# pliang279/factorized

Hardware: AMD Instinct MI355X
Metric: training samples/sec (MOSI-shape, T=20, 3 modalities) (higher is better)
Workload: dtype fp32; 1 GPU; MFM_KL_EF mosi canonical sizes, per-GPU B=32, T=20, D=325, train mode (fwd + joint loss + bwd + Adam), fp32 HIP; global_batch=32, seq_len=20, parallelism=dp1, params=477294, handover_failures=0, role_workgroups=True

## Files before the change

### factorized_amd/csrc/lstm_seq_small.hip

```cpp
#include "lstm_seq_small_dev.h"

namespace mfm {

#define MFM_SMALL_CASE(KK, BODY) case KK: BODY<KK, 4>(d, L.T, L.B, tile, lds); break;
#define MFM_SMALL_CASES(BODY) switch (d.hk4) { MFM_HK4_CASES(MFM_SMALL_CASE, BODY) default: break; }

template <bool BWD>
__global__ __launch_bounds__(1024) void lstm_seq_small_kernel(const SeqLaunch L) {
  extern __shared__ __attribute__((aligned(16))) float lds[];
  const int bid = blockIdx.x;
  MFM_SEQ_BLOCK_LSTM(L, bid, di)
  const SeqDev& d = L.d[di];
  const int tile = bid - d.block_begin;
  if (BWD) {
    MFM_SMALL_CASES(small_bwd_body)
  } else {
    MFM_SMALL_CASES(small_fwd_body)
  }
}

template <bool BWD, int R, int KS, int K0, int K1, int K2, int K3, int K4 = 0, int K5 = 0, bool BF = false>
__global__ __launch_bounds__(KS == 16 ? 1024 : 512) void lstm_seq_small_kernel4(const SeqLaunch L) {
  extern __shared__ __attribute__((aligned(16))) float lds[];
  const int bid = blockIdx.x;
// ... 73 lines not shown
template <bool BWD, int K0, int K1, int K2, int K3>
__global__ __launch_bounds__(1024) void lstm_seq_small_fold_kernel(const SeqLaunch L, const LatentDev LD, const float* __restrict__ params,
                                                                   float* __restrict__ grads) {
  extern __shared__ __attribute__((aligned(16))) float lds[];
  const int bid = blockIdx.x;
  if constexpr (!BWD) {
    if (L.n_img > 0 && bid >= L.img_begin) { wt_img_write(L.img, L.n_img, bid - L.img_begin, L.n_img_blocks); return; }
  }
  MFM_SEQ_BLOCK_LSTM(L, bid, di)
  const SeqDev& d = L.d[di];
  const int tile = bid - d.block_begin;
  if constexpr (BWD) {
    latent_bwd_row_body<false>(LD, params, grads, tile, di, lds);
    sync_stores();
  }
  MFM_TUPLE4(if (BWD) small_bwd_body<KQ, 1, 16>(d, L.T, L.B, tile, lds); else small_fwd_body<KQ, 1>(d, L.T, L.B, tile, lds))
  if constexpr (!BWD) {
    sync_stores();
    latent_fwd_row_body<false>(LD, params, tile, di, lds, true);
  }
}

template <int K0, int K1, int K2, int K3>
__global__ __launch_bounds__(1024) void lstm_seq_small_foldproj_kernel(const SeqLaunch L, const LatentDev LD, const ProjRole PR,
                                                                       const float* __restrict__ params) {
  extern __shared__ __attribute__((aligned(16))) float lds[];
  const int bid = blockIdx.x;
  const unsigned epoch = ho_epoch(PR.epoch, PR.tick);
  LSTAMP(0, 0);
  if (bid < PR.n_role) { proj_role_body(L, PR, epoch, lds); LSTAMP(0, 15); return; }
  MFM_SEQ_BLOCK_LSTM(L, bid, di)
  const SeqDev& d = L.d[di];
  const int tile = bid - d.block_begin;
  const unsigned* flg = PR.flags + (int64_t)di * L.T * PROJ_ROLE_FLAGS;
  const int ncb = PR.e[di].ncb;
  const bool pre = PR.lat_pre != 0;
  float* seq_lds = lds;
  if (pre) {
    latent_fwd_row_body<false>(LD, params, tile, di, lds, true, 1);
    seq_lds = lds + latent_fwd_lds_floats(LD.rec_size);
  }
  const float* h_lds = nullptr;
  MFM_TUPLE4(h_lds = small_fwd_body<KQ, 1, true>(d, L.T, L.B, tile, seq_lds, flg, epoch, ncb, PR.ctl))
  if (threadIdx.x < 64) {
    unsigned fv[4];
#pragma unroll
    for (int e = 0; e < 4; ++e) fv[e] = proj_flags_load(PR.flags + (int64_t)e * L.T * PROJ_ROLE_FLAGS, PR.e[e].ncb);
#pragma unroll
    for (int e = 0; e < 4; ++e) proj_flags_wait(PR.flags + (int64_t)e * L.T * PROJ_ROLE_FLAGS, fv[e], epoch, PR.e[e].ncb, PR.ctl);
  }
  LSTAMP(0, 9);
  if (pre) {
    LSTAMP(0, 8);
    latent_fwd_row_body<false>(LD, params, tile, di, lds, true, 2, h_lds, PR.lat_tail ? LD.tail_from : MFM_LAT_MAXSTAGES);
  } else {
    sync_stores();
    LSTAMP(0, 8);
    latent_fwd_row_body<false>(LD, params, tile, di, lds, true);
  }
  LSTAMP_W(0, 15);
}

template <int K0, int K1, int K2, int K3>
__global__ __launch_bounds__(1024) void lstm_seq_small_folddw_kernel(const SeqLaunch L, const LatentDev LD, const DwRole DR,
                                                                     const float* __restrict__ params, float* __restrict__ grads) {
  extern __shared__ __attribute__((aligned(16))) float lds[];
  const int bid = blockIdx.x;
  const unsigned epoch = ho_epoch(DR.epoch, DR.tick);
  LSTAMP(4, 0);
  if (bid >= 4 * L.B) {
    typedef __attribute__((address_space(4))) const char kchar;
    const char* kargs = (const char*)(kchar*)__builtin_amdgcn_kernarg_segment_ptr();
    dw_role_body(DR, epoch, lds, reinterpret_cast<const int*>(kargs + sizeof(SeqLaunch) + sizeof(LatentDev)));
    LSTAMP_W(4, 15);
    return;
  }
// ... 172 lines not shown
    if (!L.d[i].wt_img) return MFM_ERR_UNSUPPORTED;
  const int head_begin = lay_out_blocks(L, L.B), total = head_begin + 4 * L.B;
  const size_t lds_bytes = std::max(chain_lds_bytes(LD, true), small_lds_bytes(L, true, 1));
  if (lds_bytes > 160 * 1024) return MFM_ERR_UNSUPPORTED;
  return seq_launch_kernel(lstm_seq_small_decbwd_head_kernel<26, 6, 6>, "lstm_seq_small_decbwd_head_kernel", dim3(total), dim3(1024), lds_bytes, stream,
                           nullptr, L, LD, params, grads, head_begin);
}

bool seq_small_foldproj_supported(int T, int B, const int* h, const int* k, int n_enc) {
  if (opt_disabled("MFM_PROJ_FOLD") || !fold_enabled()) return false;
  if (n_enc != 4 || T < 1 || B < 1 || B > PROJ_ROLE_CB) return false;
  if (device_cus() - 4 * B < PROJ_ROLE_SLOTS) return false;
  int slots = 0, kmax = 0;
  for (int e = 0; e < 4; ++e) {
    if (k[e] < 1 || k[e] > 128 * PROJ_ROLE_MAXG) return false;
    slots += 4 * round_up(h[e], 16) / PROJ_ROLE_CB;
    if (4 * round_up(h[e], 16) / PROJ_ROLE_CB > PROJ_ROLE_FLAGS) return false;
    kmax = std::max(kmax, k[e]);
  }
  if (slots > PROJ_ROLE_SLOTS) return false;
  const int ks = proj_role_kstride(kmax);
  return ((size_t)2 * PROJ_ROLE_CB * ks + 16 * PROJ_ROLE_PW) * sizeof(float) <= 160 * 1024;
}

int seq_small_foldproj_launch(SeqLaunch& L, const LatentDev& LD, ProjRole& PR, const float* params, hipStream_t stream) {
  if (!seq_is_tuple(L, kEncHk4, 4, 0) || !chain_rows_match(LD, L.B)) return MFM_ERR_UNSUPPORTED;
  int hh[4], kk[4];
  for (int i = 0; i < 4; ++i) { hh[i] = L.d[i].h; kk[i] = PR.e[i].k; }
  if (!seq_small_foldproj_supported(L.T, L.B, hh, kk, 4)) return MFM_ERR_UNSUPPORTED;
  LSTAMP_BIND();
  int n_role = (device_cus() - 4 * L.B) / PROJ_ROLE_SLOTS * PROJ_ROLE_SLOTS;
  if (const char* e = opt_get("MFM_PROJ_FOLD_ROLES")) { const int v = atoi(e) / PROJ_ROLE_SLOTS * PROJ_ROLE_SLOTS; if (v >= PROJ_ROLE_SLOTS) n_role = v; }
  PR.n_role = n_role; PR.groups = n_role / PROJ_ROLE_SLOTS;
  int kmax = 0, cb = 0;
  for (int i = 0; i < 4; ++i) {
    kmax = std::max(kmax, PR.e[i].k);
    PR.e[i].cb_begin = cb; PR.e[i].ncb = 4 * L.d[i].Hp / PROJ_ROLE_CB;
    cb += PR.e[i].ncb;
  }
  PR.kstride = proj_role_kstride(kmax);
  const int total = lay_out_blocks(L, L.B, n_role);
  const size_t role = ((size_t)2 * PROJ_ROLE_CB * PR.kstride + 16 * PROJ_ROLE_PW) * sizeof(float);
  size_t lds_bytes = std::max(small_lds_bytes(L, false, 1), std::max(chain_lds_bytes(LD, false), role));
  PR.lat_pre = 0;
  if (!opt_disabled("MFM_LATENT_PRELOAD")) {
    bool direct = true;
    for (int i = 0; i < 4; ++i) direct = direct && (L.d[i].h & 3) == 0;
    const size_t side = chain_lds_bytes(LD, false) + small_lds_bytes(L, false, 1, true);
    if (direct && side <= 160 * 1024) { PR.lat_pre = 1; lds_bytes = std::max(side, role); }
  }
  if (!PR.lat_pre) PR.lat_tail = 0;
  if (lds_bytes > 160 * 1024) return MFM_ERR_UNSUPPORTED;
  return seq_launch_kernel(lstm_seq_small_foldproj_kernel<8, 2, 20, 30>, "lstm_seq_small_foldproj_kernel", dim3(total), dim3(1024), lds_bytes, stream, nullptr,
                           L, LD, PR, params);
}

int seq_small_fold_launch(SeqLaunch& L, bool bwd, const LatentDev& LD, const float* params, float* grads, hipStream_t stream) {
  if (!fold_enabled() || !seq_is_tuple(L, kEncHk4, 4, 0) || !chain_rows_match(LD, L.B)) return MFM_ERR_UNSUPPORTED;
  if (!((long)L.count * L.B < 6L * device_cus())) return MFM_ERR_UNSUPPORTED;
  int max_threads = 1024;
  for (int i = 0; i < 4; ++i)
    if (8 * L.d[i].Hp > max_threads) max_threads = 8 * L.d[i].Hp;
  int total = lay_out_blocks(L, L.B);
  L.n_img_blocks = 0;
  if (!bwd && L.n_img > 0) total = add_img_writers(L, total);
  const size_t lds_bytes = std::max(small_lds_bytes(L, bwd, 1), chain_lds_bytes(LD, bwd));
  if (lds_bytes > 160 * 1024) return MFM_ERR_UNSUPPORTED;
  return seq_launch_kernel(bwd ? lstm_seq_small_fold_kernel<true, 8, 2, 20, 30> : lstm_seq_small_fold_kernel<false, 8, 2, 20, 30>, "lstm_seq_small_fold_kernel",
                           dim3(total), dim3(max_threads), lds_bytes, stream, nullptr, L, LD, params, grads);
}

// ... 2 lines not shown
```

### factorized_amd/csrc/lstm_seq_small_dev.h

```cpp
#pragma once
#include <stdlib.h>

#include <algorithm>
#include <type_traits>

#include "internal.h"
#include "latent_row_dev.h"
#include "lstm_seq_dev.h"
#include "proj_role_dev.h"
#include "dw_role_dev.h"
#include "lstamp.h"

namespace mfm {

__device__ __forceinline__ void sync_stores() {
  asm volatile("s_waitcnt vmcnt(0)" ::: "memory");
  __syncthreads();
}

#ifndef MFM_SEQ_STAMP
#define MFM_SEQ_STAMP 0
#endif
#ifndef MFM_SEQ_LATE_WRITEOUT
#define MFM_SEQ_LATE_WRITEOUT 0
// ... 62 lines not shown
  } else {
    for (int i = tid; i < n; i += nt) panel[i] = (mode == 2) ? a[i] + b2[i] : a[i];
  }
}

__device__ __forceinline__ void stage_gates2(const SeqDev& d, int mode, int g, float* __restrict__ panel, int tid, int nt) {
  const int n = d.h * d.h;
  if ((n & 3) != 0) {
    stage_gate(d, mode, g, panel, tid, nt);
    stage_gate(d, mode, g + 1, panel + n, tid, nt);
    return;
  }
  const int n4 = n >> 2;
  const f32x4* a4 = reinterpret_cast<const f32x4*>((mode == 0 ? d.w_hh : d.w_ih) + (int64_t)g * n);
  const f32x4* b4 = reinterpret_cast<const f32x4*>(d.w_hh + (int64_t)g * n);
  f32x4* p4 = reinterpret_cast<f32x4*>(panel);
  for (int base = tid; base < 2 * n4; base += 8 * nt) {
    f32x4 v[8];
#pragma unroll
    for (int u = 0; u < 8; ++u) v[u] = a4[min(base + u * nt, 2 * n4 - 1)];
    if (mode == 2) {
#pragma unroll
      for (int u = 0; u < 8; ++u) v[u] += b4[min(base + u * nt, 2 * n4 - 1)];
    }
#pragma unroll
    for (int u = 0; u < 8; ++u)
      if (base + u * nt < 2 * n4) p4[base + u * nt] = v[u];
  }
}

typedef __bf16 bf16x2_t __attribute__((ext_vector_type(2)));
template <int KQ, int R, bool FLG = false, bool BF = false, bool REC = true, bool HS = false>
__device__ __forceinline__ const float* small_fwd_body(const SeqDev& d, const int T, const int B, const int tile, float* lds,
                                               const unsigned* flg = nullptr, const unsigned epoch = 0, const int ncb = 0,
                                               const HoCtl ctl = HoCtl{nullptr, nullptr, nullptr, 5000000ll, 1u},
                                               const int64_t hs_step = 0) {
  constexpr int HK = 4 * KQ;
  constexpr int HKB = (HK + 15) / 16 * 16;
  constexpr int NTH = 8 * HKB;
  constexpr int NXL = (4 * R + 7) / 8;
  constexpr int NOS = (6 * R + 7) / 8;
  const int tid = threadIdx.x, nt = blockDim.x;
  const int q = tid & 3, gp = (tid >> 2) & 1, u = tid >> 3;
  const int h = d.h, Hp = d.Hp;
  const bool dec = d.is_dec != 0;
  const bool uact = u < Hp;
  const int myrow = q & (R - 1);
  const bool rowner = q < R;
  const int b0 = tile * R;
  const int b = b0 + myrow;

  constexpr int NM = HKB / 16;
  constexpr int NWR = (R == 1) ? 4 * NM : KQ;
  constexpr int HX = (R == 1) ? HKB : HK;
  static_assert(!BF || R == 1, "bf16 dot products: one-row tiles only");
  static_assert(!HS || (!REC && !BF), "h-only record: fp32 inference bodies");
  float* hbuf = lds;
  __bf16* hb16 = reinterpret_cast<__bf16*>(lds);
  float* panel = lds + 2 * HKB * R;
  float* obuf = panel;
  float* xbuf = obuf + 2 * 6 * HKB * R;

  float w[2][NWR];
  bf16x2_t wp[2][BF ? NWR / 2 : 1];
  auto pack_w = [&]() {
    if constexpr (BF) {
#pragma unroll
      for (int gl = 0; gl < 2; ++gl)
#pragma unroll
        for (int j = 0; j < NWR / 2; ++j) wp[gl][j] = bf16x2_t{(__bf16)w[gl][2 * j], (__bf16)w[gl][2 * j + 1]};
    }
  };
  auto load_w = [&](int mode) {
    if constexpr (R == 1) {
      const float* fimg = mode == 2 ? d.wf_img : (mode == 1 ? d.wf1_img : nullptr);
      if (fimg) {
        const f32x4* img = reinterpret_cast<const f32x4*>(fimg) + (tid < NTH ? tid : 0);
#pragma unroll
        for (int gl = 0; gl < 2; ++gl)
#pragma unroll
          for (int m = 0; m < NM; ++m) {
            const f32x4 v = img[(gl * NM + m) * NTH];
#pragma unroll
            for (int i = 0; i < 4; ++i) w[gl][4 * m + i] = (tid < NTH) ? v[i] : 0.0f;
          }
        pack_w();
        return;
      }
      if ((h & 3) == 0) {
// ... 37 lines not shown
  load_w(dec ? 1 : 0);
  LSTAMP_W(dec ? 1 : 0, 1);

  float gxb[2] = {0.f, 0.f};
  if (dec && u < h) {
#pragma unroll
    for (int gl = 0; gl < 2; ++gl) gxb[gl] = d.b_ih[(2 * gp + gl) * h + u] + d.b_hh[(2 * gp + gl) * h + u];
  }
  if (dec) {
    for (int idx = tid; idx < HX * R; idx += nt) {
      const int k = idx / R, br = b0 + (idx % R);
      const float v = (k < h && br < B) ? d.h_init[(int64_t)br * d.ld_init + k] : 0.0f;
      if constexpr (BF) hb16[idx] = (__bf16)v; else hbuf[idx] = v;
    }
  }

  const int64_t row4 = 4 * (int64_t)Hp;
  const int64_t gstep = (int64_t)B * row4, sstep = (int64_t)B * Hp;
  const gfloat* xp[NXL];
  int xl[NXL];
  bool xok[NXL];
  float xpf[NXL];
#pragma unroll
  for (int i = 0; i < NXL; ++i) {
    const int e = tid + i * NTH;
    xok[i] = !dec && tid < NTH && e < 4 * HKB * R;
    const int ec = xok[i] ? e : 0;
    const int sr = ec / HKB, unit = ec % HKB, r = sr % R, g = sr / R;
    xp[i] = (const gfloat*)d.gates + ((int64_t)min(b0 + r, B - 1) * 4 + g) * Hp + unit;
    xl[i] = (g * HKB + unit) * R + r;
    xpf[i] = 0.0f;
  }
  const bool fetch_wave = FLG && !dec && (tid & ~63) < 4 * HKB * R && (tid & ~63) < NTH;
  unsigned fv = 0;
  if (!dec) {
    if constexpr (FLG) {
      if (fetch_wave) {
        const int t1 = (T > 1) ? 1 : 0;
        proj_flags_wait(flg, proj_flags_load(flg, ncb), epoch, ncb, ctl);
        proj_flags_wait(flg + t1 * PROJ_ROLE_FLAGS, proj_flags_load(flg + t1 * PROJ_ROLE_FLAGS, ncb), epoch, ncb, ctl);
        fv = proj_flags_load(flg + min(2, T - 1) * PROJ_ROLE_FLAGS, ncb);
      }
    }
#pragma unroll
    for (int i = 0; i < NXL; ++i) {
      float v0;
      if constexpr (FLG) { v0 = ld_agent((const float*)xp[i]); xpf[i] = ld_agent((const float*)xp[i] + ((T > 1) ? gstep : 0)); }
      else { v0 = xp[i][0]; xpf[i] = xp[i][(T > 1) ? gstep : 0]; }
      if (xok[i]) xbuf[xl[i]] = v0;
    }
  }
  gfloat* const p_gates = pin_s(d.gates);
  gfloat* const p_cs = pin_s(d.cs);
  gfloat* const p_hs = pin_s(d.hs);
  gfloat* op[NOS];
  int64_t ostr[NOS];
  int ol[NOS];
  bool ook[NOS];
#pragma unroll
  for (int i = 0; i < NOS; ++i) {
    const int e = tid + i * NTH;
    const bool in = tid < NTH && e < 6 * HKB * R;
    const int ec = in ? e : 0;
    const int sr = ec / HKB, unit = ec % HKB, r = sr % R, sl = sr / R;
    ook[i] = in && (b0 + r < B);
    const int br = min(b0 + r, B - 1);
    op[i] = sl < 4 ? p_gates + ((int64_t)br * 4 + sl) * Hp + unit : (sl == 4 ? p_cs : p_hs) + (int64_t)br * Hp + unit;
    ostr[i] = sl < 4 ? gstep : sstep;
    ol[i] = (sl * HKB + unit) * R + r;
  }
  gfloat* hs_p = p_hs;
  int hs_l = 0;
  bool hs_ok = false;
  if constexpr (HS) {
    const int r = tid / HKB, unit = tid - r * HKB;
    hs_ok = tid < HKB * R && b0 + r < B;
    hs_p = p_hs + (int64_t)min(b0 + r, B - 1) * Hp + (hs_ok ? unit : 0);
    hs_l = (hs_ok && unit < HX) ? unit * R + r : -1;
  }
  const int ucl = min(u, HKB - 1);
  const int my_o = (2 * gp * HKB + ucl) * R + myrow;
  const float sc0 = gp ? 2.0f : 1.0f;
// ... 67 lines not shown
            acc[1][0] = fmaf(w[1][4 * m + i], hv[m][i], acc[1][0]);
          }
#if MFM_SEQ_STAMP == 2
        asm volatile("s_memtime %0" : "=s"(st1), "+v"(acc[0][0]), "+v"(acc[1][0]) :: "memory");
#endif
      }
    } else if (dec || t > 0) {
      const float* hb = hbuf + cur * (HK * R) + q * R;
      constexpr int RING = (KQ < 4) ? KQ : 4;
      RowVec<R> ring[RING];
#pragma unroll
      for (int j = 0; j < RING; ++j) ring[j] = ld_rows<R>(hb + 4 * R * j);
#pragma unroll
      for (int j = 0; j < KQ; ++j) {
        const RowVec<R> hv = ring[j % RING];
        if (j + RING < KQ) ring[j % RING] = ld_rows<R>(hb + 4 * R * (j + RING));
#pragma unroll
        for (int gl = 0; gl < 2; ++gl)
#pragma unroll
          for (int r = 0; r < R; ++r) acc[gl][r] = fmaf(w[gl][j], hv.v[r], acc[gl][r]);
      }
    }
    if (REC && MFM_SEQ_LATE_WRITEOUT && pend) {
#pragma unroll
      for (int i = 0; i < NOS; ++i) {
        if (ook[i]) *op[i] = rprev[i];
        op[i] += ostr[i];
      }
    }
    pend = true;
    float xn[NXL];
#pragma unroll
    for (int i = 0; i < NXL; ++i) xn[i] = 0.0f;
    if (!dec) {
      const int64_t off = (int64_t)min(t + 2, T - 1) * gstep;
      if constexpr (FLG) {
        if (fetch_wave) {
          proj_flags_wait(flg + min(t + 2, T - 1) * PROJ_ROLE_FLAGS, fv, epoch, ncb, ctl);
#pragma unroll
          for (int i = 0; i < NXL; ++i) xn[i] = ld_agent((const float*)xp[i] + off);
          fv = proj_flags_load(flg + min(t + 3, T - 1) * PROJ_ROLE_FLAGS, ncb);
        }
      } else {
#pragma unroll
        for (int i = 0; i < NXL; ++i) xn[i] = xp[i][off];
      }
    }
    float mine[2];
#pragma unroll
    for (int gl = 0; gl < 2; ++gl) {
#pragma unroll
      for (int r = 0; r < R; ++r) {
        float v = acc[gl][r];
        v += dpp_f<DPP_QUAD_XOR1>(v);
        v += dpp_f<DPP_QUAD_XOR2>(v);
        acc[gl][r] = v;
      }
      mine[gl] = sel_row<R>(acc[gl], myrow) + (gl ? gx1 : gx0);
    }
    const float a0 = act_scaled(mine[0], sc0);
    const float a1 = act_sigmoid(mine[1]);
    const float p0 = dpp_xor4(a0), p1 = dpp_xor4(a1);
    const float gf = gp ? p1 : a1, go = gp ? a1 : p1;
    c = fmaf(gf, c, a0 * p0);
    float hv = go * act_tanh(c);
#if MFM_SEQ_STAMP == 3
    asm volatile("s_memtime %0" : "=s"(st1), "+v"(hv), "+v"(c) :: "memory");
#endif
    if (uact && rowner) {
      if constexpr (REC) {
        float* ob = obuf + par * (6 * HKB * R) + my_o;
        ob[0] = a0; ob[HKB * R] = a1;
        ob[(4 - gp) * HKB * R] = gp ? hv : c;
      }
      if (gp == 0 && u < HX) {
        const float hn = (b < B) ? hv : 0.0f;
        if constexpr (BF) hb16[(cur ^ 1) * HX + u] = (__bf16)hn; else hbuf[(cur ^ 1) * (HX * R) + u * R + myrow] = hn;
      }
    }
    if (!dec) {
#pragma unroll
      for (int i = 0; i < NXL; ++i)
        if (xok[i]) xbuf[(par ^ 1) * (4 * HKB * R) + xl[i]] = xpf[i];
    }
#if MFM_SEQ_STAMP == 4
    asm volatile("s_waitcnt lgkmcnt(0)" ::: "memory");
    st1 = seq_clock();
#endif
    lds_barrier();
#if MFM_SEQ_STAMP == 5
    st1 = seq_clock();
#endif
#if MFM_SEQ_STAMP
    if (MFM_SEQ_STAMP != 6 && t >= 1) { asm volatile("s_waitcnt lgkmcnt(0)" ::: "memory"); st_sum += st1 - st0; }
#endif
    if (REC && !MFM_SEQ_LATE_WRITEOUT) {
#pragma unroll
      for (int i = 0; i < NOS; ++i) {
        if (ook[i]) *op[i] = obuf[par * (6 * HKB * R) + ol[i]];
        op[i] += ostr[i];
      }
      pend = false;
    }
    if constexpr (HS) {
      if (hs_ok) *hs_p = hs_l >= 0 ? hbuf[(cur ^ 1) * (HX * R) + hs_l] : 0.0f;
      hs_p += hs_step;
    }
#pragma unroll
    for (int i = 0; i < NXL; ++i) xpf[i] = xn[i];
    cur ^= 1;
  };
  auto flush = [&](const int t_last) {
    if (!REC || !pend) return;
#pragma unroll
    for (int i = 0; i < NOS; ++i) {
      if (ook[i]) *op[i] = obuf[(t_last & 1) * (6 * HKB * R) + ol[i]];
      op[i] += ostr[i];
    }
    pend = false;
  };
  if (dec) {
    step(0);
    flush(0);
    LSTAMP(1, 3);
    if (T > 1) {
      __syncthreads();
      load_w(2);
      LSTAMP_W(1, 4);
      for (int t = 1; t < T; ++t) step(t);
      flush(T - 1);
    }
  } else {
    for (int t = 0; t < T; ++t) step(t);
    flush(T - 1);
  }
  LSTAMP(dec ? 1 : 0, 7);
#if MFM_SEQ_STAMP
  __syncthreads();
  if (blockIdx.x == 0 && (tid & 63) == 0 && T > 2) {
    const int nsteps = (MFM_SEQ_STAMP == 6) ? T - 2 : T - 1;
    p_cs[(int64_t)(T - 1) * sstep + (tid >> 6)] = (float)((double)st_sum / (double)nsteps);
  }
// ... 357 lines not shown
```

### factorized_amd/csrc/plan_build.hip

```cpp
#include "plan_internal.h"

namespace mfm {

PIdx pidx_for(int variant) {
  PIdx p;
  memset(&p, 0xff, sizeof(p));
  p.enc[0] = 0; p.enc[1] = 6; p.enc[2] = 12;
  p.dec[0] = 18; p.dec[1] = 24; p.dec[2] = 30;
  if (variant == 0) {
    p.enc[3] = 36;
    p.to_z[3] = 42; p.to_lv[3] = 44; p.to_z[0] = 46; p.to_z[1] = 48; p.to_z[2] = 50;
    p.to_lv[0] = 52; p.to_lv[1] = 54; p.to_lv[2] = 56;
    p.zf1[3] = 58; p.zf2[3] = 60; p.zf1[0] = 62; p.zf2[0] = 64; p.zf1[1] = 66; p.zf2[1] = 68; p.zf1[2] = 70; p.zf2[2] = 72;
    p.y_f1 = 74; p.y_f2 = 76; p.count = 78;
    return p;
  }
  p.mfl[0] = 36; p.mfl[1] = 40; p.mfl[2] = 44;
  p.att1_1 = 48; p.att1_2 = 50; p.att2_1 = 52; p.att2_2 = 54; p.g1_1 = 56; p.g1_2 = 58; p.g2_1 = 60; p.g2_2 = 62;
  p.to_z[3] = 68;
  int next = 70;
  if (variant == 1) {
    p.to_lv[3] = 70; p.to_z[0] = 72; p.to_z[1] = 74; p.to_z[2] = 76; p.to_lv[0] = 78; p.to_lv[1] = 80; p.to_lv[2] = 82;
    next = 84;
  }
// ... 344 lines not shown
      }
      L.bias_tab = fits ? 1 : 0;
    }
    L.bias_n = 0;
    for (int ch = 0; ch < L.nch && L.bias_tab; ++ch) {
      int cnt = 0;
      for (int i = 0; i < L.nops; ++i) if (L.nch == 1 || P->lat_ops[i].chain == ch) cnt += P->lat_ops[i].N;
      L.bias_n = std::max(L.bias_n, cnt);
    }
    L.pre = 0;
    if (const char* e = opt_get("MFM_LATENT_PRE")) L.pre = (atoi(e) != 0 && L.nch > 1 && L.nstages <= 6) ? 1 : 0;
    for (int ch = 0; ch < L.nch && L.pre; ++ch)
      for (int st = 0; st < L.nstages; ++st)
        if (L.nitems_fwd_c[ch][st] > 512 || L.nitems_bwd_c[ch][st] > 512) L.pre = 0;
    L.row_threads = MFM_LAT_ROW_THREADS;
    if (L.nch > 1) {
      int mx = 0;
      for (int ch = 0; ch < L.nch; ++ch)
        for (int st = 0; st < L.nstages; ++st) mx = std::max(mx, std::max(L.nitems_fwd_c[ch][st], L.nitems_bwd_c[ch][st]));
      int in_sum = 0;
      for (int e = 0; e < 4; ++e) in_sum += L.enc_n[e];
      if (mx <= 512 && in_sum <= 512) L.row_threads = 512;
    }
    if (L.nch > 1)
      for (int st = 0; st < L.nstages; ++st) {
        int sn = 0, sk = 0;
        for (int i = L.stage_begin[st]; i < L.stage_begin[st + 1]; ++i) { sn += P->lat_ops[i].N; sk += P->lat_ops[i].K; }
        L.nitems_fwd[st] = 4 * sn; L.nitems_bwd[st] = 4 * sk;
      }
  }

  P->lat_ops_off = carve(cur, (int64_t)(sizeof(P->lat_ops) / (sizeof(float))));
  P->pf_flags = (V == 0) ? carve(cur, (int64_t)4 * P->T * PROJ_ROLE_FLAGS) : -1;
  if ((long)(P->n_enc > 3 ? P->n_enc : 3) * c.B < 6L * device_cus() && !P->seq_bf16) {
    for (int i = 0; i < P->n_enc + 3; ++i) {
      const int hh = i < P->n_enc ? P->enc[i].h : P->dec[i - P->n_enc].h;
      if (hh > MFM_SEQ_MAX_RESIDENT_H) continue;
      const int64_t HKB = round_up(4 * round_up(cdiv(hh, 4), 2), 16);
      P->wt_img[i] = carve(cur, 4 * HKB * HKB);
      if (i >= P->n_enc && (hh & 3) == 0) { P->wf_img[i - P->n_enc] = carve(cur, 4 * HKB * HKB); P->wf_img[3 + i - P->n_enc] = carve(cur, 4 * HKB * HKB); }
    }
  }
  if (V == 0 && c.B <= DWR_ROWS) {
    P->dw_flags = carve(cur, (int64_t)4 * P->T * DWR_ROWS + 4 * DWR_ROWS);
    P->dw_table = carve(cur, (int64_t)DWR_TABLE_CAP * 4);
  }
  P->lat_items_off = carve(cur, (int64_t)P->lat_items.size());
  P->lat_grd = carve(cur, (int64_t)c.B * rs);
  P->lat_rec = carve(cur, (int64_t)c.B * rs);
  P->lat_seed = (V == 2) ? carve(cur, (int64_t)c.B * rs) : -1;
  {
    long minb = 48;
    if (const char* e = opt_get("MFM_MMD_GEMM_MINB")) minb = atol(e);
    P->mmd_scr = (V == 2 && minb > 0 && c.B >= minb && c.B <= 8192) ? carve(cur, mmd_scratch_floats(c.B, 4)) : -1;
  }
  if (V != 0) P->dh_last[3] = carve(cur, (int64_t)c.B * P->nzy);
  P->yhat = carve(cur, (int64_t)c.B * c.output_dim);
  P->ones = carve(cur, TB);
  P->losses = carve(cur, 64);
  P->ws_floats = cur;
  return MFM_OK;
}

}
```

### factorized_amd/csrc/plan_forward.hip

```cpp
#include "plan_internal.h"

namespace mfm {

__global__ void tick_kernel(unsigned long long* t64, unsigned* t32) {
  if (threadIdx.x == 0 && blockIdx.x == 0) {
    if (t64) *t64 += 1ull;
    if (t32) *t32 += 1u;
  }
}
__global__ void guard_propagate_kernel(const unsigned* status, float* guard) {
  if (threadIdx.x == 0 && blockIdx.x == 0 && *status != 0u) *guard = __builtin_nanf("");
}
bool stream_capturing(hipStream_t s) {
  hipStreamCaptureStatus st = hipStreamCaptureStatusNone;
  if (hipStreamIsCapturing(s, &st) != hipSuccess) { (void)hipGetLastError(); return false; }
  return st == hipStreamCaptureStatusActive;
}

MfmSeqDesc seq_desc(const MfmPlan* P, const SeqBuf& sb, int pbase, const float* params, float* W, bool dec) {
  MfmSeqDesc d;
  memset(&d, 0, sizeof(d));
  d.gates = W + sb.gates; d.hs = W + sb.hs; d.cs = W + sb.cs;
  d.w_ih = params + P->off[pbase + W_IH];
  d.w_hh = params + P->off[pbase + W_HH];
// ... 54 lines not shown
      PL.ngroups = P->n_enc;
      for (int e = 0; e < P->n_enc; ++e) {
        const SeqBuf& sb = P->enc[e];
        const int pb = P->enc_p[e];
        PanelGroup& G = PL.g[e];
        G.w = params + P->off[pb + W_IH]; G.ldw = P->enc_d[e];
        G.bias = params + P->off[pb + B_IH]; G.bias2 = params + P->off[pb + B_HH];
        G.n = 4 * sb.Hp; G.seg = sb.Hp; G.seg_valid = sb.h; G.k_off = P->enc_xoff[e]; G.k_len = P->enc_d[e];
      }
      const int rc0 = proj_pack_prepare(PL, P->pj, W + P->pj_wimg, W + P->pj_bimg, &PJD);
      if (rc0 != MFM_OK) return rc0;
      pjp = &PJD; P->pj_pack_call = P->calls;
    }
    if (st16 && train && !(xhat_out && (xhat_out[0] || xhat_out[1] || xhat_out[2]))) {
      DecFc1LargeLaunch FLp;
      memset(&FLp, 0, sizeof(FLp));
      FLp.n_items = 3; FLp.rows = (int)TB;
      for (int m = 0; m < 3; ++m) {
        DecFc1LargeItem& I = FLp.it[m];
        I.w = params + P->off[P->dec_p[m] + FC_W]; I.d = P->dec_d[m]; I.h = P->dec[m].h; I.Hp = P->dec[m].Hp;
        I.ld_dxhat = P->dxh_ld[m]; I.ldx = P->D; I.wimg = W + P->fc1_wimg[m];
      }
      if (dec_fc1_large_uses_wimg(FLp)) {
        const int rc0 = fc1_pack_prepare(FLp, &FCA);
        if (rc0 != MFM_OK) return rc0;
        fcp = &FCA; P->fc1_pack_call = P->calls;
      }
    }
    RUN(K_PACK, pack_all_launch(&PKL, pjp, fcp, s));
  }

  bool proj_in_fold = false;
  const bool capturing = stream_capturing(s);
  if (V == 0 && !seq_bf16 && !st16 && P->n_enc == 4 && P->fold_state >= 0 && P->projfold_state >= 0 && P->pf_flags >= 0 &&
      P->opt_handover && TB * P->D < ((int64_t)1 << 28)) {
    int hh[4], kk[4];
    for (int e = 0; e < 4; ++e) { hh[e] = P->enc[e].h; kk[e] = P->enc_d[e]; }
    proj_in_fold = seq_small_foldproj_supported(T, B, hh, kk, 4);
    if (!proj_in_fold) P->projfold_state = -1;
  }
  auto run_f0 = [&]() -> int {
    MfmGemmDesc g[6];
    memset(g, 0, sizeof(g));
    for (int e = 0; e < P->n_enc; ++e) {
      const SeqBuf& sb = P->enc[e];
      const int pb = P->enc_p[e];
      MfmGemmDesc& d = g[e];
      d.a = x + P->enc_xoff[e]; d.a_sm = P->D; d.a_sk = 1; d.a_sz = 0;
      d.b = params + P->off[pb + W_IH]; d.b_sz = (int64_t)sb.h * P->enc_d[e]; d.b_sn = P->enc_d[e]; d.b_sk = 1;
      d.c = W + sb.gates; d.c_sz = sb.Hp; d.ldc = 4 * (int64_t)sb.Hp;
      d.c_bf16 = st16 ? 1 : 0;
      d.bias = params + P->off[pb + B_IH]; d.bias2 = params + P->off[pb + B_HH]; d.bias_sz = sb.h;
      d.m = (int)TB; d.n = sb.Hp; d.n_valid = sb.h; d.k = P->enc_d[e]; d.batch = 4; d.split_k = 1;
      d.alpha = 1.0f;
    }
    const char* pe = opt_get("MFM_PANEL_MINROWS");
    const bool panel_forced = pe && TB >= atol(pe);
    const bool panel = (pe ? panel_forced : TB >= 16L * device_cus()) && P->n_enc <= MFM_PANEL_MAXG && (int64_t)TB * P->D < ((int64_t)1 << 29);
    if (panel || (st16 && P->proj16)) {
      PanelLaunch PL;
      memset(&PL, 0, sizeof(PL));
      PL.a = x; PL.lda = P->D; PL.M = (int)TB; PL.K = P->D;
      for (int e = 0; e < P->n_enc; ++e) {
        const SeqBuf& sb = P->enc[e];
        const int pb = P->enc_p[e];
        PanelGroup& G = PL.g[PL.ngroups++];
        G.w = params + P->off[pb + W_IH]; G.ldw = P->enc_d[e];
// ... 43 lines not shown
          I.w_hh = sum ? params + P->off[pb + W_HH] : nullptr; I.w_ih = params + P->off[pb + W_IH];
          I.img = W + P->wf_img[sum ? m : 3 + m]; I.h = P->dec[m].h;
          I.HKB = round_up(4 * round_up(cdiv(P->dec[m].h, 4), 2), 16);
          I.fwd = 1;
        }
      }
    }
  }
  LatentDev L = P->lat;
  {
    L.ops = reinterpret_cast<const LatOp*>(W + P->lat_ops_off);
    L.items_fwd = reinterpret_cast<const int*>(W + P->lat_items_off);
    L.items_bwd = L.items_fwd + (size_t)4 * MFM_LAT_MAXSTAGES * MFM_LAT_ROW_THREADS * 4;
    for (int e = 0; e < 4; ++e) {
      if (e == 3 && V != 0) { L.enc_h[e] = W + P->zyin; L.enc_ld[e] = P->nzy; continue; }
      L.enc_h[e] = st16 ? W + P->h_last[e] : W + P->enc[e].hs + (int64_t)(T - 1) * B * P->enc[e].Hp;
      L.enc_ld[e] = P->enc[e].Hp;
    }
    for (int m = 0; m < 3; ++m) { L.dec_init[m] = W + P->dec_init[m]; L.dec_ld[m] = P->dec_h[m]; }
    L.rec = W + P->lat_rec;
    L.yhat_out = yhat_out ? yhat_out : W + P->yhat;
    L.y = y; L.losses = losses; L.train = train;
    L.seed = seed * 0x9E3779B97F4A7C15ull + P->calls * 0xD1B54A32D192ED03ull;
    L.tick = reinterpret_cast<const unsigned long long*>(P->tick_ptr(W));
  }
  bool folded = false;
  if (proj_in_fold) {
    MfmSeqDesc q[4];
    for (int e = 0; e < 4; ++e) q[e] = seq_desc(P, P->enc[e], P->enc_p[e], params, W, false);
    ProjRole PR;
    memset(&PR, 0, sizeof(PR));
    PR.x = x; PR.ldx = P->D; PR.x_rows = (int)TB;
    PR.flags = reinterpret_cast<unsigned*>(W + P->pf_flags); PR.epoch = epoch_base(P->calls); PR.tick = P->tick_ptr(W);
    PR.ctl = P->ho_ctl(W, losses + 4, 1u);
    PR.fault = (P->opt_fault == 1) ? 1 : 0;
    if (PR.fault) P->opt_fault = 0;
    PR.zs = zs;
    PR.loss_ptr = zs.ptr[0]; PR.loss_n = (int)zs.n[0];
    PR.bf16 = c.precision ? 1 : 0;
    if (n_wt_items == 7) { for (int i = 0; i < 7; ++i) PR.wt[i] = wt_items[i]; PR.n_wt = 7; }
    if (!opt_disabled("MFM_WF_IMG")) {
      for (int k = 0; k < 6; ++k) {
        const int m = k % 3;
        const bool sum = k >= 3;
        if (P->wf_img[m] < 0 || P->wf_img[3 + m] < 0 || T < 2) continue;
        WtImgItem& I = PR.wf[PR.n_wf++];
        const int pb = P->dec_p[m];
        I.w_hh = sum ? params + P->off[pb + W_HH] : nullptr; I.w_ih = params + P->off[pb + W_IH];
        I.img = W + P->wf_img[sum ? m : 3 + m]; I.h = P->dec[m].h;
        I.HKB = round_up(4 * round_up(cdiv(P->dec[m].h, 4), 2), 16);
      }
    }
    PR.zs.ptr[0] = nullptr; PR.zs.n[0] = 0;
    for (int e = 0; e < 4; ++e) {
      const int pb = P->enc_p[e];
      PR.e[e].w = params + P->off[pb + W_IH]; PR.e[e].b_ih = params + P->off[pb + B_IH]; PR.e[e].b_hh = params + P->off[pb + B_HH];
      PR.e[e].k_off = P->enc_xoff[e]; PR.e[e].k = P->enc_d[e];
    }
    {
      const int dech[3] = {P->dec[0].h, P->dec[1].h, P->dec[2].h};
      PR.lat_tail = seq_small_dectail_supported(T, B, dech, L) ? 1 : 0;
    }
    int rc;
    { Timer _t(P, s, K_ENC_FWD); rc = seq_foldproj_launch(q, 4, T, B, L, params, PR, s); }
    if (rc == MFM_OK) { folded = true; P->projfold_state = 1; P->fold_state = 1; P->ever_handover = true; if (PR.n_wt) P->wt_call = P->calls;
                        if (PR.n_wf == 6) P->wf_call = P->calls;
// ... 149 lines not shown
```

### factorized_amd/csrc/plan_internal.h

```cpp
#pragma once
#include <math.h>
#include <stdlib.h>

#include <algorithm>
#include <new>
#include <vector>

#include "internal.h"
#include "proj_role_dev.h"
#include "dw_role_dev.h"
#include "pack_dev.h"
#include "lstm_seq_dev.h"

namespace mfm {

enum KernelId {
  K_PROJ = 0, K_ENC_FWD, K_LAT_FWD, K_DEC_FWD, K_FC1_FWD, K_MSE, K_FC1_BWD, K_DEC_BWD, K_DEC_DW,
  K_LAT_BWD, K_ENC_BWD, K_ENC_DW, K_ADAM, K_LAT_DW, K_PACK,
  K_MFN_GLUE, K_MFN_ATT_FWD, K_MFN_MEM_FWD, K_MFN_HEADS, K_MFN_MEM_BWD, K_MFN_ATT_BWD, K_MMD, K_COUNT
};

struct PIdx {
  int enc[4], dec[3];
  int mfl[3];
// ... 20 lines not shown
  int64_t n_params;
  int D, T, B;
  int n_enc;
  int enc_d[6], enc_xoff[6], enc_h[6], enc_p[6];
  int dec_d[3], dec_h[3], dec_p[3], dec_xoff[3];
  mfm::SeqBuf enc[6], dec[3];
  int64_t dec_dhs[3], dec_init[3], dec_dinit[3], xhat[3], dxhat[3];
  int64_t lat_rec, dh_last[4], yhat, ones, losses;
  int tot, A2, nzy;
  int64_t dcx[3];
  int64_t cstar, h1, m1, att, attended, h2, m2, chat, a1, a2, gam1, gam2, mems, mem_out;
  int64_t zero_blk, zero_len;
  int64_t dhs_blk, dhs_len;
  int64_t zyin, d_hT, dmem, datt;
  int64_t du1, du2, dchat, dh2, dlog, dh1, dcs;
  int64_t lat_seed;
  int64_t mmd_scr;
  int z_seg[4];
  const float* gauss;
  int64_t ws_floats;
  mfm::LatentDev lat;
  mfm::LatOp lat_ops[MFM_LAT_MAXOPS];
  int64_t lat_ops_off, lat_grd, lat_items_off;
  int lay_f1[4], lay_m1[4], lay_c1, lay_mc;
  std::vector<int> lat_items;
  int timing_mask, timing_every;
  std::vector<mfm::TimingPair> pool;
  size_t pool_used;
  uint64_t calls;
  const float* grads_prezeroed;
  int fold_state = 0;
  int projfold_state = 0;
  int64_t pf_flags = -1;
  int64_t wt_img[mfm::MFM_WT_MAX] = {-1, -1, -1, -1, -1, -1, -1, -1, -1};
  unsigned long long wt_call = ~0ull;
  int64_t wf_img[6] = {-1, -1, -1, -1, -1, -1};
  unsigned long long wf_call = ~0ull;
  unsigned long long lat_tail_call = ~0ull;
  int dwfold_state = 0;
  int64_t dw_flags = -1, dw_table = -1;
  std::vector<int> dw_table_host;
  unsigned dw_epoch = 0;
  int dw_table_key = -1;
  const float* dw_table_ws = nullptr;
  bool seq_bf16 = false;
  bool st16 = false;
  int64_t h_last[6];
  int64_t x16; int x16_ld, x16_off[3];
  int dxh_ld[3];
  int64_t fc1_wimg[3];
  bool proj16 = false;
  mfm::ProjPlan pj;
  int64_t pj_wimg, pj_bimg;
  unsigned long long x16_call = ~0ull;
  int64_t dwb_slabs = -1, dwb_slab_floats = 0;
  unsigned long long pj_pack_call = ~0ull, fc1_pack_call = ~0ull;
  unsigned long long fc1_bwd_call = ~0ull;
  mfm::OptTable* opts = nullptr;
  int opt_handover = 1;
  int64_t opt_timeout_us = 50000;
  int64_t opt_guard = -1;
  int opt_fault = 0;
  int opt_bf16_dot = 0;
  bool ever_handover = false;
  unsigned* host_status = nullptr;
  static constexpr int ST_STATUS = MFM_LOSS_SLOTS, ST_TICK = MFM_LOSS_SLOTS + 2, ST_DW_TICK = MFM_LOSS_SLOTS + 4;
// ... 75 lines not shown
```

### factorized_amd/csrc/proj_role_dev.h

```cpp
#pragma once
#include "internal.h"
#include "lstm_seq_dev.h"
#include "lstamp.h"

namespace mfm {

constexpr int PROJ_ROLE_CB = 32;
constexpr int PROJ_ROLE_SLOTS = 32;
constexpr int PROJ_ROLE_MAXG = 4;
constexpr int PROJ_ROLE_FLAGS = 16;
constexpr int PROJ_ROLE_PW = 4 * 96 + 4;

struct ProjRoleEnc { const float* w; const float* b_ih; const float* b_hh; int k_off, k, cb_begin, ncb; };
constexpr int PROJ_ROLE_WT = 7;
struct HoCtl { unsigned* status; unsigned* host; float* poison; long long timeout; unsigned bit; };
__device__ __forceinline__ void ho_give_up(const HoCtl& c) {
  if ((threadIdx.x & 63) == 0) {
    if (c.status) __hip_atomic_fetch_or(c.status, c.bit, __ATOMIC_RELAXED, __HIP_MEMORY_SCOPE_AGENT);
    if (c.host) __hip_atomic_store(c.host + (c.bit >> 1), c.bit, __ATOMIC_RELAXED, __HIP_MEMORY_SCOPE_SYSTEM);
    if (c.poison) __hip_atomic_store(c.poison, __builtin_nanf(""), __ATOMIC_RELAXED, __HIP_MEMORY_SCOPE_AGENT);
  }
}
__device__ __forceinline__ unsigned ho_epoch(unsigned base, const unsigned* tick) {
  const unsigned e = base + (tick ? *tick : 0u);
  return e ? e : 0x5bd1e995u;
}

struct ProjRole {
  const float* x; int ldx; int x_rows;
  int n_role, groups, kstride;
  unsigned* flags; unsigned epoch;
  const unsigned* tick;
  HoCtl ctl;
  int fault;
  int lat_pre;
  int lat_tail;
  float* loss_ptr; int loss_n;
  int bf16;
  ProjRoleEnc e[4];
  ZeroSpans zs;
  WtImgItem wt[PROJ_ROLE_WT]; int n_wt;
  WtImgItem wf[6]; int n_wf;
};

static inline int proj_role_kstride(int k) { int s4 = ((k + 15) / 16 * 16) / 4; if ((s4 & 1) == 0) ++s4; return 4 * s4; }

__device__ __forceinline__ void st_agent(float* p, float v) { __hip_atomic_store(p, v, __ATOMIC_RELAXED, __HIP_MEMORY_SCOPE_AGENT); }
__device__ __forceinline__ float ld_agent(const float* p) { return __hip_atomic_load(p, __ATOMIC_RELAXED, __HIP_MEMORY_SCOPE_AGENT); }
__device__ __forceinline__ unsigned ld_agent_u(const unsigned* p) { return __hip_atomic_load(p, __ATOMIC_RELAXED, __HIP_MEMORY_SCOPE_AGENT); }

__device__ __forceinline__ bool proj_flags_ready(unsigned v, unsigned epoch, int ncb) {
  const int lane = threadIdx.x & 63;
  return __builtin_amdgcn_ballot_w64(lane < ncb && v != epoch) == 0ull;
}
__device__ __forceinline__ unsigned proj_flags_load(const unsigned* f, int ncb) {
  const int lane = threadIdx.x & 63;
  return ld_agent_u(f + (lane < ncb ? lane : 0));
}
__device__ __forceinline__ void proj_flags_wait(const unsigned* f, unsigned v, unsigned epoch, int ncb, const HoCtl& ctl) {
  if (proj_flags_ready(v, epoch, ncb)) return;
  const long long t0 = wall_clock64();
  do {
    __builtin_amdgcn_s_sleep(2);
    v = proj_flags_load(f, ncb);
    if (wall_clock64() - t0 >= ctl.timeout) { ho_give_up(ctl); return; }
  } while (!proj_flags_ready(v, epoch, ncb));
}

__device__ __forceinline__ void proj_role_body(const SeqLaunch& L, const ProjRole& PR, const unsigned epoch, float* lds) {
  const int tid = threadIdx.x, lane = tid & 63, wave = tid >> 6;
  const int r = blockIdx.x;
  const int slot = r & (PROJ_ROLE_SLOTS - 1), grp = r >> 5;
  const int T = L.T, B = L.B;
  int e = -1;
#pragma unroll
  for (int i = 0; i < 4; ++i)
    if (slot >= PR.e[i].cb_begin && slot < PR.e[i].cb_begin + PR.e[i].ncb) e = i;

  if (e >= 0 && grp < T) {
    const ProjRoleEnc& E = PR.e[e];
    const SeqDev& d = L.d[e];
    const int K = E.k, h = d.h, Hp = d.Hp;
// ... 37 lines not shown
        if (lrow[j] < PROJ_ROLE_CB) *reinterpret_cast<f32x4*>(img + lrow[j] * ks + 4 * lgr[j]) = zero_tail(rv[j], lgr[j]);
    };

    f32x4 rw[PROJ_ROLE_MAXG], rx[PROJ_ROLE_MAXG];
#pragma unroll
    for (int j = 0; j < PROJ_ROLE_MAXG; ++j) {
      const int gc = col0 + lrow[j];
      const int g = gc / Hp, u = gc - g * Hp;
      const bool ok = lrow[j] < PROJ_ROLE_CB && u < h && 4 * lgr[j] < K;
      const int off = ok ? (((g * h + u) * K + 4 * lgr[j]) * 4) : -16;
      rw[j] = __builtin_bit_cast(f32x4, __builtin_amdgcn_raw_buffer_load_b128(wres, off, 0, 0));
    }
    load_x(grp, rx);
    const int orow = tid >> 5, ocol = tid & 31;
    float bias = 0.0f;
    bool cvalid;
    {
      const int gc = col0 + ocol;
      const int g = gc / Hp, u = gc - g * Hp;
      cvalid = u < h;
      if (cvalid) bias = E.b_ih[g * h + u] + E.b_hh[g * h + u];
    }
    if (grp == 0 && tid < PR.loss_n) st_agent(PR.loss_ptr + tid, 0.0f);
    park(Ws, rw);
    park(Xs, rx);
    __syncthreads();
    LSTAMP(0, 1);

    const int bi = lane & 15, q = lane >> 4;
    const int frag = wave >> 2, kpart = wave & 3;
    const int fr = frag >> 1, fc = frag & 1;
    const int NG16 = G >> 2;
    const int pw0 = (((orow >> 4) * 2 + (ocol >> 4)) * 4) * PROJ_ROLE_PW + (orow & 3) * 96 + (ocol & 15) + 16 * ((orow & 15) >> 2);
    float* const out = d.gates;
    const int64_t orow_stride = 4 * (int64_t)Hp;
    for (int t = grp; t < T; t += PR.groups) {
      const int tn = t + PR.groups;
      if (tn < T) load_x(tn, rx);
      const float* xa = Xs + (16 * fr + bi) * ks + 4 * q;
      const float* wb = Ws + (16 * fc + bi) * ks + 4 * q;
      f32x4 acc = {0.f, 0.f, 0.f, 0.f};
      for (int g16 = kpart; g16 < NG16; g16 += 4) {
        const f32x4 a = *reinterpret_cast<const f32x4*>(xa + 16 * g16);
        const f32x4 b = *reinterpret_cast<const f32x4*>(wb + 16 * g16);
#pragma unroll
        for (int c = 0; c < 4; ++c) acc = mma16x16x4(a[c], b[c], acc);
      }
#pragma unroll
      for (int c = 0; c < 4; ++c) Ps[wave * PROJ_ROLE_PW + c * 96 + lane] = acc[c];
      __syncthreads();
      if (orow < B) {
        const float v = Ps[pw0] + Ps[pw0 + PROJ_ROLE_PW] + Ps[pw0 + 2 * PROJ_ROLE_PW] + Ps[pw0 + 3 * PROJ_ROLE_PW];
        st_agent(out + ((int64_t)t * B + orow) * orow_stride + col0 + ocol, cvalid ? v + bias : 0.0f);
      }
      if (tn < T) park(Xs, rx);
      asm volatile("s_waitcnt vmcnt(0)" ::: "memory");
      __syncthreads();
      if (tid == 0 && !(PR.fault && r == 0 && t == grp))
        __hip_atomic_store(PR.flags + ((int64_t)e * T + t) * PROJ_ROLE_FLAGS + cbl, epoch, __ATOMIC_RELAXED, __HIP_MEMORY_SCOPE_AGENT);
      LSTAMP(0, 16 + (t - grp) / PR.groups);
    }
  }
  LSTAMP(0, 12);
  wf_img_write(PR.wf, PR.n_wf, r, PR.n_role);
  wt_img_write(PR.wt, PR.n_wt, r, PR.n_role);
  LSTAMP(0, 13);
  const f32x4 z4 = {0.f, 0.f, 0.f, 0.f};
#pragma unroll 1
  for (int s = 0; s < MFM_GEMM_ZSPANS; ++s) {
    f32x4* p = reinterpret_cast<f32x4*>(PR.zs.ptr[s]);
    const int64_t n4 = PR.zs.n[s] >> 2;
    for (int64_t i = (int64_t)r * 1024 + tid; i < n4; i += (int64_t)PR.n_role * 1024) p[i] = z4;
  }
}

}
```

Measured before the change: 227,200 samples/s.

## Replace per-step projection flags with epoch-tagged 64-bit value words

The projection role now writes each gate pre-activation as a 64-bit word carrying the epoch in its high half, and the LSTM consumer polls those words directly instead of waiting on separate per-timestep flag arrays. This removes the store-drain wait and flag store on every timestep except the first, and lets the consumer skip a separate flag load per step. In exchange it allocates an extra workspace buffer, doubles the width of each handover value, and adds a wave-wide ballot poll on the data itself. The later wait on all four encoders' flags still relies on flags that are now only published for t=0.

```diff
diff --git a/factorized_amd/csrc/lstm_seq_small.hip b/factorized_amd/csrc/lstm_seq_small.hip
--- a/factorized_amd/csrc/lstm_seq_small.hip
+++ b/factorized_amd/csrc/lstm_seq_small.hip
@@ -129,8 +129,7 @@
   MFM_SEQ_BLOCK_LSTM(L, bid, di)
   const SeqDev& d = L.d[di];
   const int tile = bid - d.block_begin;
-  const unsigned* flg = PR.flags + (int64_t)di * L.T * PROJ_ROLE_FLAGS;
-  const int ncb = PR.e[di].ncb;
+  const unsigned long long* pw = PR.words + PR.e[di].w_off;
   const bool pre = PR.lat_pre != 0;
   float* seq_lds = lds;
   if (pre) {
@@ -138,7 +137,7 @@
     seq_lds = lds + latent_fwd_lds_floats(LD.rec_size);
   }
   const float* h_lds = nullptr;
-  MFM_TUPLE4(h_lds = small_fwd_body<KQ, 1, true>(d, L.T, L.B, tile, seq_lds, flg, epoch, ncb, PR.ctl))
+  MFM_TUPLE4(h_lds = small_fwd_body<KQ, 1, true>(d, L.T, L.B, tile, seq_lds, pw, epoch, PR.w_ld, PR.ctl))
   if (threadIdx.x < 64) {
     unsigned fv[4];
 #pragma unroll
@@ -377,11 +376,14 @@
   int n_role = (device_cus() - 4 * L.B) / PROJ_ROLE_SLOTS * PROJ_ROLE_SLOTS;
   if (const char* e = opt_get("MFM_PROJ_FOLD_ROLES")) { const int v = atoi(e) / PROJ_ROLE_SLOTS * PROJ_ROLE_SLOTS; if (v >= PROJ_ROLE_SLOTS) n_role = v; }
   PR.n_role = n_role; PR.groups = n_role / PROJ_ROLE_SLOTS;
+  if (!PR.words || ((uintptr_t)PR.words & 7) != 0) return MFM_ERR_UNSUPPORTED;
   int kmax = 0, cb = 0;
+  PR.w_ld = 0;
   for (int i = 0; i < 4; ++i) {
     kmax = std::max(kmax, PR.e[i].k);
     PR.e[i].cb_begin = cb; PR.e[i].ncb = 4 * L.d[i].Hp / PROJ_ROLE_CB;
     cb += PR.e[i].ncb;
+    PR.e[i].w_off = PR.w_ld; PR.w_ld += 4 * L.d[i].Hp;
   }
   PR.kstride = proj_role_kstride(kmax);
   const int total = lay_out_blocks(L, L.B, n_role);
diff --git a/factorized_amd/csrc/lstm_seq_small_dev.h b/factorized_amd/csrc/lstm_seq_small_dev.h
--- a/factorized_amd/csrc/lstm_seq_small_dev.h
+++ b/factorized_amd/csrc/lstm_seq_small_dev.h
@@ -118,7 +118,7 @@
 typedef __bf16 bf16x2_t __attribute__((ext_vector_type(2)));
 template <int KQ, int R, bool FLG = false, bool BF = false, bool REC = true, bool HS = false>
 __device__ __forceinline__ const float* small_fwd_body(const SeqDev& d, const int T, const int B, const int tile, float* lds,
-                                               const unsigned* flg = nullptr, const unsigned epoch = 0, const int ncb = 0,
+                                               const unsigned long long* pw = nullptr, const unsigned epoch = 0, const int pw_ld = 0,
                                                const HoCtl ctl = HoCtl{nullptr, nullptr, nullptr, 5000000ll, 1u},
                                                const int64_t hs_step = 0) {
   constexpr int HK = 4 * KQ;
@@ -141,6 +141,7 @@
   constexpr int HX = (R == 1) ? HKB : HK;
   static_assert(!BF || R == 1, "bf16 dot products: one-row tiles only");
   static_assert(!HS || (!REC && !BF), "h-only record: fp32 inference bodies");
+  static_assert(!FLG || R == 1, "projection words: one-row tiles only (one word per fetching lane)");
   float* hbuf = lds;
   __bf16* hb16 = reinterpret_cast<__bf16*>(lds);
   float* panel = lds + 2 * HKB * R;
@@ -244,22 +245,36 @@
     xpf[i] = 0.0f;
   }
   const bool fetch_wave = FLG && !dec && (tid & ~63) < 4 * HKB * R && (tid & ~63) < NTH;
-  unsigned fv = 0;
+  const int64_t wstep = (int64_t)B * pw_ld;
+  const gu64* xw[NXL];
+  unsigned long long xpw[NXL];
+#pragma unroll
+  for (int i = 0; i < NXL; ++i) {
+    xw[i] = nullptr; xpw[i] = 0ull;
+    if constexpr (FLG) {
+      const int ec = xok[i] ? tid + i * NTH : 0;
+      const int sr = ec / HKB, unit = ec % HKB, r = sr % R, g = sr / R;
+      xw[i] = (const gu64*)pw + (int64_t)min(b0 + r, B - 1) * pw_ld + g * Hp + unit;
+    }
+  }
   if (!dec) {
     if constexpr (FLG) {
       if (fetch_wave) {
-        const int t1 = (T > 1) ? 1 : 0;
-        proj_flags_wait(flg, proj_flags_load(flg, ncb), epoch, ncb, ctl);
-        proj_flags_wait(flg + t1 * PROJ_ROLE_FLAGS, proj_flags_load(flg + t1 * PROJ_ROLE_FLAGS, ncb), epoch, ncb, ctl);
-        fv = proj_flags_load(flg + min(2, T - 1) * PROJ_ROLE_FLAGS, ncb);
-      }
-    }
-#pragma unroll
-    for (int i = 0; i < NXL; ++i) {
-      float v0;
-      if constexpr (FLG) { v0 = ld_agent((const float*)xp[i]); xpf[i] = ld_agent((const float*)xp[i] + ((T > 1) ? gstep : 0)); }
-      else { v0 = xp[i][0]; xpf[i] = xp[i][(T > 1) ? gstep : 0]; }
-      if (xok[i]) xbuf[xl[i]] = v0;
+        unsigned long long w0[NXL];
+#pragma unroll
+        for (int i = 0; i < NXL; ++i) { w0[i] = ld_word(xw[i]); xpw[i] = ld_word(xw[i] + ((T > 1) ? wstep : 0)); }
+        proj_words_wait(xw, 0, w0, xok, epoch, ctl);
+#pragma unroll
+        for (int i = 0; i < NXL; ++i)
+          if (xok[i]) xbuf[xl[i]] = word_value(w0[i]);
+      }
+    } else {
+#pragma unroll
+      for (int i = 0; i < NXL; ++i) {
+        const float v0 = xp[i][0];
+        xpf[i] = xp[i][(T > 1) ? gstep : 0];
+        if (xok[i]) xbuf[xl[i]] = v0;
+      }
     }
   }
   gfloat* const p_gates = pin_s(d.gates);
@@ -393,16 +408,17 @@
     float xn[NXL];
 #pragma unroll
     for (int i = 0; i < NXL; ++i) xn[i] = 0.0f;
+    unsigned long long xnw[NXL];
+#pragma unroll
+    for (int i = 0; i < NXL; ++i) xnw[i] = 0ull;
     if (!dec) {
-      const int64_t off = (int64_t)min(t + 2, T - 1) * gstep;
       if constexpr (FLG) {
         if (fetch_wave) {
-          proj_flags_wait(flg + min(t + 2, T - 1) * PROJ_ROLE_FLAGS, fv, epoch, ncb, ctl);
-#pragma unroll
-          for (int i = 0; i < NXL; ++i) xn[i] = ld_agent((const float*)xp[i] + off);
-          fv = proj_flags_load(flg + min(t + 3, T - 1) * PROJ_ROLE_FLAGS, ncb);
+#pragma unroll
+          for (int i = 0; i < NXL; ++i) xnw[i] = ld_word(xw[i] + (int64_t)min(t + 2, T - 1) * wstep);
         }
       } else {
+        const int64_t off = (int64_t)min(t + 2, T - 1) * gstep;
 #pragma unroll
         for (int i = 0; i < NXL; ++i) xn[i] = xp[i][off];
       }
@@ -440,6 +456,11 @@
       }
     }
     if (!dec) {
+      if constexpr (FLG) {
+        if (fetch_wave) proj_words_wait(xw, (int64_t)min(t + 1, T - 1) * wstep, xpw, xok, epoch, ctl);
+#pragma unroll
+        for (int i = 0; i < NXL; ++i) xpf[i] = word_value(xpw[i]);
+      }
 #pragma unroll
       for (int i = 0; i < NXL; ++i)
         if (xok[i]) xbuf[(par ^ 1) * (4 * HKB * R) + xl[i]] = xpf[i];
@@ -468,7 +489,7 @@
       hs_p += hs_step;
     }
 #pragma unroll
-    for (int i = 0; i < NXL; ++i) xpf[i] = xn[i];
+    for (int i = 0; i < NXL; ++i) { xpf[i] = xn[i]; xpw[i] = xnw[i]; }
     cur ^= 1;
   };
   auto flush = [&](const int t_last) {
diff --git a/factorized_amd/csrc/plan_build.hip b/factorized_amd/csrc/plan_build.hip
--- a/factorized_amd/csrc/plan_build.hip
+++ b/factorized_amd/csrc/plan_build.hip
@@ -400,6 +400,11 @@
 
   P->lat_ops_off = carve(cur, (int64_t)(sizeof(P->lat_ops) / (sizeof(float))));
   P->pf_flags = (V == 0) ? carve(cur, (int64_t)4 * P->T * PROJ_ROLE_FLAGS) : -1;
+  if (V == 0 && P->n_enc == 4 && c.B <= PROJ_ROLE_CB) {
+    int64_t cols = 0;
+    for (int e = 0; e < 4; ++e) cols += 4 * (int64_t)P->enc[e].Hp;
+    P->pf_words = carve(cur, 2 * (int64_t)P->T * c.B * cols);
+  }
   if ((long)(P->n_enc > 3 ? P->n_enc : 3) * c.B < 6L * device_cus() && !P->seq_bf16) {
     for (int i = 0; i < P->n_enc + 3; ++i) {
       const int hh = i < P->n_enc ? P->enc[i].h : P->dec[i - P->n_enc].h;
diff --git a/factorized_amd/csrc/plan_forward.hip b/factorized_amd/csrc/plan_forward.hip
--- a/factorized_amd/csrc/plan_forward.hip
+++ b/factorized_amd/csrc/plan_forward.hip
@@ -110,7 +110,7 @@
 
   bool proj_in_fold = false;
   const bool capturing = stream_capturing(s);
-  if (V == 0 && !seq_bf16 && !st16 && P->n_enc == 4 && P->fold_state >= 0 && P->projfold_state >= 0 && P->pf_flags >= 0 &&
+  if (V == 0 && !seq_bf16 && !st16 && P->n_enc == 4 && P->fold_state >= 0 && P->projfold_state >= 0 && P->pf_flags >= 0 && P->pf_words >= 0 &&
       P->opt_handover && TB * P->D < ((int64_t)1 << 28)) {
     int hh[4], kk[4];
     for (int e = 0; e < 4; ++e) { hh[e] = P->enc[e].h; kk[e] = P->enc_d[e]; }
@@ -220,6 +220,7 @@
     memset(&PR, 0, sizeof(PR));
     PR.x = x; PR.ldx = P->D; PR.x_rows = (int)TB;
     PR.flags = reinterpret_cast<unsigned*>(W + P->pf_flags); PR.epoch = epoch_base(P->calls); PR.tick = P->tick_ptr(W);
+    PR.words = reinterpret_cast<unsigned long long*>(W + P->pf_words);
     PR.ctl = P->ho_ctl(W, losses + 4, 1u);
     PR.fault = (P->opt_fault == 1) ? 1 : 0;
     if (PR.fault) P->opt_fault = 0;
diff --git a/factorized_amd/csrc/plan_internal.h b/factorized_amd/csrc/plan_internal.h
--- a/factorized_amd/csrc/plan_internal.h
+++ b/factorized_amd/csrc/plan_internal.h
@@ -76,6 +76,7 @@
   int fold_state = 0;
   int projfold_state = 0;
   int64_t pf_flags = -1;
+  int64_t pf_words = -1;
   int64_t wt_img[mfm::MFM_WT_MAX] = {-1, -1, -1, -1, -1, -1, -1, -1, -1};
   unsigned long long wt_call = ~0ull;
   int64_t wf_img[6] = {-1, -1, -1, -1, -1, -1};
diff --git a/factorized_amd/csrc/proj_role_dev.h b/factorized_amd/csrc/proj_role_dev.h
--- a/factorized_amd/csrc/proj_role_dev.h
+++ b/factorized_amd/csrc/proj_role_dev.h
@@ -11,7 +11,7 @@
 constexpr int PROJ_ROLE_FLAGS = 16;
 constexpr int PROJ_ROLE_PW = 4 * 96 + 4;
 
-struct ProjRoleEnc { const float* w; const float* b_ih; const float* b_hh; int k_off, k, cb_begin, ncb; };
+struct ProjRoleEnc { const float* w; const float* b_ih; const float* b_hh; int k_off, k, cb_begin, ncb, w_off; };
 constexpr int PROJ_ROLE_WT = 7;
 struct HoCtl { unsigned* status; unsigned* host; float* poison; long long timeout; unsigned bit; };
 __device__ __forceinline__ void ho_give_up(const HoCtl& c) {
@@ -30,6 +30,7 @@
   const float* x; int ldx; int x_rows;
   int n_role, groups, kstride;
   unsigned* flags; unsigned epoch;
+  unsigned long long* words; int w_ld;
   const unsigned* tick;
   HoCtl ctl;
   int fault;
@@ -46,8 +47,32 @@
 static inline int proj_role_kstride(int k) { int s4 = ((k + 15) / 16 * 16) / 4; if ((s4 & 1) == 0) ++s4; return 4 * s4; }
 
 __device__ __forceinline__ void st_agent(float* p, float v) { __hip_atomic_store(p, v, __ATOMIC_RELAXED, __HIP_MEMORY_SCOPE_AGENT); }
-__device__ __forceinline__ float ld_agent(const float* p) { return __hip_atomic_load(p, __ATOMIC_RELAXED, __HIP_MEMORY_SCOPE_AGENT); }
 __device__ __forceinline__ unsigned ld_agent_u(const unsigned* p) { return __hip_atomic_load(p, __ATOMIC_RELAXED, __HIP_MEMORY_SCOPE_AGENT); }
+
+typedef __attribute__((address_space(1))) unsigned long long gu64;
+__device__ __forceinline__ void st_word(gu64* p, float v, unsigned epoch) {
+  __hip_atomic_store(p, ((unsigned long long)epoch << 32) | __builtin_bit_cast(unsigned, v), __ATOMIC_RELAXED, __HIP_MEMORY_SCOPE_AGENT);
+}
+__device__ __forceinline__ unsigned long long ld_word(const gu64* p) { return __hip_atomic_load(p, __ATOMIC_RELAXED, __HIP_MEMORY_SCOPE_AGENT); }
+__device__ __forceinline__ float word_value(unsigned long long w) { return __builtin_bit_cast(float, (unsigned)w); }
+template <int N>
+__device__ __forceinline__ void proj_words_wait(const gu64* const (&p)[N], const int64_t off, unsigned long long (&w)[N], const bool (&act)[N],
+                                                const unsigned epoch, const HoCtl& ctl) {
+  auto stale = [&]() {
+    bool s = false;
+#pragma unroll
+    for (int i = 0; i < N; ++i) s = s || (act[i] && (unsigned)(w[i] >> 32) != epoch);
+    return __builtin_amdgcn_ballot_w64(s) != 0ull;
+  };
+  if (!stale()) return;
+  const long long t0 = wall_clock64();
+  do {
+    __builtin_amdgcn_s_sleep(2);
+#pragma unroll
+    for (int i = 0; i < N; ++i) w[i] = ld_word(p[i] + off);
+    if (wall_clock64() - t0 >= ctl.timeout) { ho_give_up(ctl); return; }
+  } while (stale());
+}
 
 __device__ __forceinline__ bool proj_flags_ready(unsigned v, unsigned epoch, int ncb) {
   const int lane = threadIdx.x & 63;
@@ -151,8 +176,7 @@
     const int fr = frag >> 1, fc = frag & 1;
     const int NG16 = G >> 2;
     const int pw0 = (((orow >> 4) * 2 + (ocol >> 4)) * 4) * PROJ_ROLE_PW + (orow & 3) * 96 + (ocol & 15) + 16 * ((orow & 15) >> 2);
-    float* const out = d.gates;
-    const int64_t orow_stride = 4 * (int64_t)Hp;
+    gu64* const out = (gu64*)PR.words + E.w_off + col0 + ocol;
     for (int t = grp; t < T; t += PR.groups) {
       const int tn = t + PR.groups;
       if (tn < T) load_x(tn, rx);
@@ -168,14 +192,15 @@
 #pragma unroll
       for (int c = 0; c < 4; ++c) Ps[wave * PROJ_ROLE_PW + c * 96 + lane] = acc[c];
       __syncthreads();
-      if (orow < B) {
+      const bool withheld = PR.fault && r == 0 && t == grp;
+      if (orow < B && !withheld) {
         const float v = Ps[pw0] + Ps[pw0 + PROJ_ROLE_PW] + Ps[pw0 + 2 * PROJ_ROLE_PW] + Ps[pw0 + 3 * PROJ_ROLE_PW];
-        st_agent(out + ((int64_t)t * B + orow) * orow_stride + col0 + ocol, cvalid ? v + bias : 0.0f);
+        st_word(out + ((int64_t)t * B + orow) * PR.w_ld, cvalid ? v + bias : 0.0f, epoch);
       }
       if (tn < T) park(Xs, rx);
-      asm volatile("s_waitcnt vmcnt(0)" ::: "memory");
+      if (t == 0) asm volatile("s_waitcnt vmcnt(0)" ::: "memory");
       __syncthreads();
-      if (tid == 0 && !(PR.fault && r == 0 && t == grp))
+      if (t == 0 && tid == 0 && !withheld)
         __hip_atomic_store(PR.flags + ((int64_t)e * T + t) * PROJ_ROLE_FLAGS + cbl, epoch, __ATOMIC_RELAXED, __HIP_MEMORY_SCOPE_AGENT);
       LSTAMP(0, 16 + (t - grp) / PR.groups);
     }
```

Measured after the change: 231,900 samples/s, median of 6. +2.1%, better.
